# githubpradeep/llm_np_cp

Hardware: AMD Instinct MI355X
Metric: decode tokens/sec (higher is better)
Workload: dtype bf16; 1 GPU; model=llama-3.2-1b, kv_dtype=bf16, global_batch=1, seq_len=867, parallelism=tp1

## Files before the change

### csrc/llm_ops.hip

```cpp

#include <hip/hip_runtime.h>
#include <cstdint>
#include <cstdio>
#include <cstdlib>
#include <type_traits>

#include "common.h"


#define GEMV_ROWS_PER_BLOCK 4
#define STAGE_RAW 0
#define STAGE_NORM 1
#define STAGE_GLU 2
#define STAGE_NORM2 3
#define STAGE_NORM_EMBED 4

DEVINL u16 glu_act(float xx, float u, int act) {
  float a;
  if (act == 0) {
    a = xx / (1.f + __expf(-xx));
  } else {
    float c = 0.7978845608028654f * (xx + 0.044715f * xx * xx * xx);
    a = 0.5f * xx * (1.f + tanhf(c));
  }
// ... 1643 lines not shown
      sc[w] = (mls[w * 2] == -INFINITY) ? 0.f : __expf(mls[w * 2] - mt);
      lt += mls[w * 2 + 1] * sc[w];
    }
    float inv = 1.f / lt;
    for (int d = lane; d < hd; d += 64) {
      float v = 0.f;
#pragma unroll
      for (int w = 0; w < 4; w++) v += accs[w * hd + d] * sc[w];
      out[((size_t)m * nh + h) * hd + d] = f2b(v * inv);
    }
  }
}


template <bool KV8>
DEVINL void attn_dec_body(char* smem, const int chunk, const int SPLIT,
                          const u16* __restrict__ qkv, void* __restrict__ kc,
                          void* __restrict__ vc, u16* __restrict__ out,
                          const int* __restrict__ len_ptr,
                          const float* __restrict__ cost,
                          const float* __restrict__ sint,
                          float* __restrict__ kS, float* __restrict__ vS,
                          float* __restrict__ scratch, int* __restrict__ cnt,
                          int nh, int kvh, int hd, int S, float scale,
                          float softcap, int window) {
  float* red = (float*)smem;
  int* lastflag = (int*)(red + 4 * hd + 8);

  const int h = blockIdx.x;
  const int b = blockIdx.z;
  qkv += (size_t)b * (nh + 2 * kvh) * hd;
  out += (size_t)b * nh * hd;
  kc = (char*)kc + (size_t)b * kvh * S * hd * (KV8 ? 1 : 2);
  vc = (char*)vc + (size_t)b * kvh * S * hd * (KV8 ? 1 : 2);
  if (KV8) { kS += (size_t)b * kvh * S; vS += (size_t)b * kvh * S; }
  scratch += (size_t)b * nh * SPLIT * (hd + 2);
  cnt += b * nh;
  const int grp = nh / kvh;
  const int kvhead = h / grp;
  const int pos = len_ptr[b];
  int start = 0;
  if (window > 0 && pos + 1 - window > 0) start = pos + 1 - window;
  const int hist = pos - start;
  const int clen = (hist + SPLIT - 1) / SPLIT;
  const int c0 = start + chunk * clen;
  const int c1 = min(c0 + clen, pos);
  const bool last_chunk = (chunk == SPLIT - 1);

  const int LP = hd / 8;
  const int PP = 64 / LP;
  const int wave = threadIdx.x >> 6, lane = threadIdx.x & 63;
  const int p = lane / LP, d0 = (lane % LP) * 8;
  const int hd2 = hd / 2;
  const float* cp = cost + (size_t)pos * hd2;
  const float* sp = sint + (size_t)pos * hd2;

  const u16* qh = qkv + (size_t)h * hd;
  const u16* kh = qkv + (size_t)(nh + kvhead) * hd;
  const u16* vh = qkv + (size_t)(nh + kvh + kvhead) * hd;
  const u16* K0 = (const u16*)kc + (size_t)kvhead * S * hd;
  const u16* V0 = (const u16*)vc + (size_t)kvhead * S * hd;
  const uint8_t* K08 = (const uint8_t*)kc + (size_t)kvhead * S * hd;
  const uint8_t* V08 = (const uint8_t*)vc + (size_t)kvhead * S * hd;
  const float* kS0 = KV8 ? kS + (size_t)kvhead * S : nullptr;
  const float* vS0 = KV8 ? vS + (size_t)kvhead * S : nullptr;

// ... 174 lines not shown
    mrun = mn;
  }

  float* accs = red;
  float* mls = red + 4 * hd;
  if (lane < LP) {
#pragma unroll
    for (int j = 0; j < 8; j++) accs[wave * hd + d0 + j] = acc[j];
  }
  if (lane == 0) {
    mls[wave * 2] = mrun;
    mls[wave * 2 + 1] = lrun;
  }
  __syncthreads();

  float* part = scratch + ((size_t)h * SPLIT + chunk) * (hd + 2);
  if (wave == 0) {
    float mt = fmaxf(fmaxf(mls[0], mls[2]), fmaxf(mls[4], mls[6]));
    float lt = 0.f, sc[4];
#pragma unroll
    for (int w = 0; w < 4; w++) {
      sc[w] = (mls[w * 2] == -INFINITY) ? 0.f : __expf(mls[w * 2] - mt);
      lt += mls[w * 2 + 1] * sc[w];
    }
    if (SPLIT == 1) {
      float inv = 1.f / lt;
      for (int d = lane; d < hd; d += 64) {
        float v = 0.f;
#pragma unroll
        for (int w = 0; w < 4; w++) v += accs[w * hd + d] * sc[w];
        out[(size_t)h * hd + d] = f2b(v * inv);
      }
    } else {
      for (int d = lane; d < hd; d += 64) {
        float v = 0.f;
#pragma unroll
        for (int w = 0; w < 4; w++) v += accs[w * hd + d] * sc[w];
        part[2 + d] = v;
      }
      if (lane == 0) { part[0] = mt; part[1] = lt; }
    }
  }
  if (SPLIT == 1) return;

  asm volatile("s_waitcnt vmcnt(0)" ::: "memory");
  __syncthreads();
  if (threadIdx.x == 0) {
    __builtin_amdgcn_fence(__ATOMIC_RELEASE, "agent");
    asm volatile("s_waitcnt vmcnt(0)" ::: "memory");
    int t = __hip_atomic_fetch_add(&cnt[h], 1, __ATOMIC_RELAXED,
                                   __HIP_MEMORY_SCOPE_AGENT);
    *lastflag = (t == SPLIT - 1);
  }
  __syncthreads();
  if (!*lastflag) return;

  if (threadIdx.x == 0)
    __builtin_amdgcn_fence(__ATOMIC_ACQUIRE, "agent");
  __syncthreads();
  if (wave == 0) {
    const float* base = scratch + (size_t)h * SPLIT * (hd + 2);
    float mt = -INFINITY;
    for (int c = 0; c < SPLIT; c++)
      mt = fmaxf(mt, base[(size_t)c * (hd + 2)]);
    float lt = 0.f;
    for (int c = 0; c < SPLIT; c++) {
      float mc = base[(size_t)c * (hd + 2)];
      if (mc != -INFINITY)
        lt += base[(size_t)c * (hd + 2) + 1] * __expf(mc - mt);
    }
    float inv = 1.f / lt;
    for (int d = lane; d < hd; d += 64) {
      float v = 0.f;
      for (int c = 0; c < SPLIT; c++) {
        float mc = base[(size_t)c * (hd + 2)];
        if (mc != -INFINITY)
          v += base[(size_t)c * (hd + 2) + 2 + d] * __expf(mc - mt);
      }
      out[(size_t)h * hd + d] = f2b(v * inv);
    }
  }
  __syncthreads();
  if (threadIdx.x == 0) cnt[h] = 0;
}


struct AttnPf {
  const void* ptr[4];
  long bytes[4];
  long stride0;
  float* sink;
  int never;
};

constexpr int PF_LD = 8;
constexpr int PF_TRIP = 256 * PF_LD;

template <typename F>
// ... 2 lines not shown
#pragma unroll
  for (int j = 0; j < PF_LD; j++) {
    long s = seg(j * 256 + (int)threadIdx.x);
    s = s < nseg ? s : nseg - 1;
    v[j] = base[s];
  }
  uint32_t a = 0;
#pragma unroll
  for (int j = 0; j < PF_LD; j++) {
    asm volatile("" ::"v"(v[j]));
    a ^= v[j][0];
  }
  return a;
}

DEVINL void attn_dec_prefetch(const AttnPf& pf, const int split) {
  const uint32_t nx = gridDim.x;
  const uint32_t pfy = gridDim.y - split;
  const uint32_t npb = nx * pfy * gridDim.z;
  const uint32_t pb =
      (blockIdx.z * pfy + (blockIdx.y - split)) * nx + blockIdx.x;
  uint32_t acc = 0;
  uint32_t g0 = 0;
#pragma unroll
  for (int r = 0; r < 4; r++) {
    const u4v* base = (const u4v*)pf.ptr[r];
    const long nseg = pf.bytes[r] >> 4;
    if (base == nullptr || nseg <= 0) continue;
    const long spu = pf.stride0 >> 4;
    if (r == 0 && spu > 0 && (nx & 7) == 0 && nseg < (1l << 31)) {
      const uint32_t c = blockIdx.x & 7;
      const uint32_t nunit = (uint32_t)((nseg + spu - 1) / spu);
      if (nunit <= c) continue;
      const uint32_t uspu = (uint32_t)spu;
      const long vseg = (long)((nunit - c + 7) / 8) * spu;
      const uint32_t rc = (pb / nx) * (nx / 8) + blockIdx.x / 8;
// ... 36 lines not shown
  extern __shared__ __attribute__((aligned(16))) char smem[];
  int SPLIT = gridDim.y;
  if constexpr (PF) {
    const AttnPfLaunch& a = (pfa, ...);
    if ((int)blockIdx.y >= a.split) {
      attn_dec_prefetch(a.pf, a.split);
      return;
    }
    SPLIT = a.split;
  }
  attn_dec_body<KV8>(smem, blockIdx.y, SPLIT, qkv, kc, vc, out, len_ptr, cost,
                     sint, kS, vS, scratch, cnt, nh, kvh, hd, S, scale,
                     softcap, window);
}

static hipError_t attn_dec_launch(const void* qkv, void* kc, void* vc,
                                  void* out, const void* len_ptr,
                                  const void* cost, const void* sint,
                                  void* kS, void* vS, int kv8, void* scratch,
                                  void* cnt, int split, int batch, int nh,
                                  int kvh, int hd, int S, float scale,
                                  float softcap, int window, int pf_blocks,
                                  const AttnPf& pf, hipStream_t stream) {
  size_t lds = (4 * hd + 8) * sizeof(float) + 16;
  const int pfy = pf_blocks > 0 ? (pf_blocks + nh - 1) / nh : 0;
#define ATTN_DEC_ARGS                                                        \
  (const u16*)qkv, kc, vc, (u16*)out, (const int*)len_ptr,                   \
      (const float*)cost, (const float*)sint, (float*)kS, (float*)vS,        \
      (float*)scratch, (int*)cnt, nh, kvh, hd, S, scale, softcap, window
#define ATTN_DEC_CASE(KV8V)                                                  \
  hipLaunchKernelGGL((k_attn_dec_t<KV8V, false>), dim3(nh, split, batch),    \
                     dim3(256), lds, stream, ATTN_DEC_ARGS)
#define ATTN_DEC_PF_CASE(KV8V)                                               \
  hipLaunchKernelGGL((k_attn_dec_t<KV8V, true, AttnPfLaunch>),               \
                     dim3(nh, split + pfy, batch), dim3(256), lds, stream,   \
                     ATTN_DEC_ARGS, AttnPfLaunch{split, pf})
  if (pfy > 0) {
    if (kv8) ATTN_DEC_PF_CASE(true);
    else ATTN_DEC_PF_CASE(false);
  } else {
    if (kv8) ATTN_DEC_CASE(true);
    else ATTN_DEC_CASE(false);
  }
#undef ATTN_DEC_PF_CASE
#undef ATTN_DEC_ARGS
#undef ATTN_DEC_CASE
  return hipGetLastError();
}

extern "C" hipError_t launch_attn_dec_pf(
    const void* qkv, void* kc, void* vc, void* out, const void* len_ptr,
    const void* cost, const void* sint, void* kS, void* vS, int kv8,
    void* scratch, void* cnt, int split, int batch, int nh, int kvh, int hd,
    int S, float scale, float softcap, int window, int pf_blocks,
    const void* p0, long n0, const void* p1, long n1, const void* p2,
    long n2, const void* p3, long n3, long stride0, void* sink,
    hipStream_t stream) {
  AttnPf pf{{p0, p1, p2, p3}, {n0, n1, n2, n3}, stride0, (float*)sink, -1};
  if (pf_blocks > 0 && sink == nullptr) return hipErrorInvalidValue;
  return attn_dec_launch(qkv, kc, vc, out, len_ptr, cost, sint, kS, vS, kv8,
                         scratch, cnt, split, batch, nh, kvh, hd, S, scale,
                         softcap, window, pf_blocks, pf, stream);
}

extern "C" hipError_t launch_attn_dec(const void* qkv, void* kc, void* vc,
                                      void* out, const void* len_ptr,
                                      const void* cost, const void* sint,
                                      void* kS, void* vS, int kv8,
                                      void* scratch, void* cnt, int split,
                                      int batch,
                                      int nh, int kvh, int hd, int S,
                                      float scale, float softcap, int window,
                                      hipStream_t stream) {
  return attn_dec_launch(qkv, kc, vc, out, len_ptr, cost, sint, kS, vS, kv8,
                         scratch, cnt, split, batch, nh, kvh, hd, S, scale,
                         softcap, window, 0, AttnPf{}, stream);
}


typedef short b4v __attribute__((ext_vector_type(4)));

template <int HD, bool KV8>
__global__ void __launch_bounds__(64)
k_attn_prefill_mfma(const u16* __restrict__ q, const void* __restrict__ kc,
                    const void* __restrict__ vc, u16* __restrict__ out,
                    const int* __restrict__ len_ptr,
                    const float* __restrict__ kS,
                    const float* __restrict__ vS, int M, int nh, int kvh,
                    int S, float scale, float softcap, int window) {
  constexpr int HD32 = HD / 32;
  constexpr int HD16 = HD / 16;
// ... 240 lines not shown
DEVINL uint32_t fkey(float f) {
  union { float f; uint32_t u; } c; c.f = f;
  return (c.u & 0x80000000u) ? ~c.u : (c.u ^ 0x80000000u);
}
DEVINL float fkey_inv(uint32_t k) {
  union { float f; uint32_t u; } c;
  c.u = (k & 0x80000000u) ? (k ^ 0x80000000u) : ~k;
  return c.f;
}

DEVINL uint64_t pack_ki(uint32_t key, int idx) {
  return ((uint64_t)key << 32) | (uint32_t)(0x7fffffff - idx);
}
DEVINL int unpack_idx(uint64_t p) { return 0x7fffffff - (int)(uint32_t)p; }

DEVINL void logit_max_body(const void* __restrict__ logits, int V, int lbf16,
                           unsigned long long* __restrict__ gmax) {
  const int b = blockIdx.y;
  gmax += b;
  const float* lf = (const float*)logits + (size_t)b * V;
  const u16* lh = (const u16*)logits + (size_t)b * V;
  float mv = -INFINITY;
  int mi = 0;
  for (int i = blockIdx.x * 256 + threadIdx.x; i < V; i += gridDim.x * 256) {
    float v = lbf16 ? b2f(lh[i]) : lf[i];
    if (v > mv || (v == mv && i < mi)) { mv = v; mi = i; }
  }
  uint64_t pk = pack_ki(fkey(mv), mi);
#pragma unroll
  for (int w = 1; w < 64; w <<= 1) {
    uint64_t o = __shfl_xor((unsigned long long)pk, w);
    if (o > pk) pk = o;
  }
  __shared__ unsigned long long ws[4];
  if ((threadIdx.x & 63) == 0) ws[threadIdx.x >> 6] = pk;
  __syncthreads();
  if (threadIdx.x == 0) {
    uint64_t b = ws[0];
    for (int w = 1; w < 4; w++) if (ws[w] > b) b = ws[w];
    atomicMax(gmax, (unsigned long long)b);
  }
}
// ... 94 lines not shown
  gmax += b; pick += b; cnt += b; nout += b;
  out_ring += (size_t)b * ring_stride;
  const float* lf = (const float*)logits + (size_t)b * V;
  const u16* lh = (const u16*)logits + (size_t)b * V;
  float thresh = -INFINITY;
  uint32_t tau = 0;
  if (SEL) {
    sel += (size_t)b * SEL_WORDS;
    tau = (uint32_t)sel[SEL_TAU];
  } else if (!greedy) {
    thresh = fkey_inv((uint32_t)(*gmax >> 32)) + __logf(min_p) / inv_temp;
  }
  const uint32_t c = (uint32_t)(*ctr) ^ ((uint32_t)b * 0x85ebca6bu);
  float bv = -INFINITY;
  int bi = 0x7fffffff;
  for (int i = blockIdx.x * 256 + threadIdx.x; i < V; i += gridDim.x * 256) {
    float v = lbf16 ? b2f(lh[i]) : lf[i];
    if (SEL ? (fkey(v) < tau) : (v < thresh)) continue;
    float sc = v;
    if (!greedy) {
      uint32_t r = hash32(hash32((uint32_t)i ^ (c * 0x9e3779b9u)) ^
                          (uint32_t)seed);
      float u = (r + 1.0f) * 2.3283064e-10f;
      sc = v * inv_temp - __logf(-__logf(u));
    }
    if (sc > bv || (sc == bv && i < bi)) { bv = sc; bi = i; }
  }
  sample_pick_commit(bv, bi, V, gmax, pick, cnt, next_token, out_ring, nout,
                     len_ptr, bump_len, SEL ? sel : nullptr);
}

extern "C" __global__ void __launch_bounds__(256)
k_sample_pick(const void* __restrict__ logits, int V, int lbf16,
              long ring_stride, float min_p,
              int greedy, uint64_t seed, float inv_temp,
              unsigned long long* __restrict__ gmax,
              uint64_t* __restrict__ ctr,
              unsigned long long* __restrict__ pick,
              int* __restrict__ cnt, int* __restrict__ next_token,
              int* __restrict__ out_ring, int* __restrict__ nout,
              int* __restrict__ len_ptr, int bump_len) {
  sample_pick_body<false>(logits, V, lbf16, ring_stride, min_p, greedy, seed,
// ... 46 lines not shown
             __logf(__uint_as_float(samp[SAMP_MINP])) / inv_temp;
  if (MINP && selected) {
    const float min_p = __uint_as_float(samp[SAMP_MINP]);
    if (min_p > 0.0f) {
      float cut = fkey_inv((uint32_t)(*gmax >> 32)) + __logf(min_p) / inv_temp;
      if (cut == 0.0f) cut = -0.0f;
      const uint32_t kc = fkey(cut);
      if (kc > tau) tau = kc;
    }
  }
  const uint32_t k0 =
      hash32(hash32(samp[SAMP_CTR] ^ 0x9e3779b9u) ^ samp[SAMP_SEED]);
  const uint32_t k1 = hash32(k0 ^ samp[SAMP_SEED + 1] ^ 0x85ebca6bu);
  float bv = -INFINITY;
  int bi = 0x7fffffff;
  for (int i = blockIdx.x * 256 + threadIdx.x; i < V; i += gridDim.x * 256) {
    float v = lbf16 ? b2f(lh[i]) : lf[i];
    if (selected ? (fkey(v) < tau) : (v < thresh)) continue;
    float sc = v;
    if (!greedy) {
      uint32_t r = hash32(hash32((uint32_t)i ^ k0) ^ k1);
      float u = (r + 1.0f) * 2.3283064e-10f;
      sc = v * inv_temp - __logf(-__logf(u));
    }
    if (sc > bv || (sc == bv && i < bi)) { bv = sc; bi = i; }
  }
  sample_pick_commit(bv, bi, V, gmax, pick, cnt, next_token, out_ring, nout,
                     len_ptr, bump_len, selected ? sel : nullptr);
}

template <bool PHASE2>
DEVINL void sample_select_body(
    const void* __restrict__ logits, int V, int lbf16,
    int top_k, float top_p, float inv_temp, int shift,
    int last, const unsigned long long* __restrict__ gmax,
    unsigned long long* __restrict__ sel) {
  const int b = blockIdx.y;
  const int t = threadIdx.x;
  sel += (size_t)b * SEL_WORDS;
  unsigned long long* hist = sel + SEL_HIST;
  const float* lf = (const float*)logits + (size_t)b * V;
// ... 108 lines not shown
}

extern "C" __global__ void __launch_bounds__(256)
k_sample_select_rows2(const void* __restrict__ logits, int V, int lbf16,
                      const uint32_t* __restrict__ samp, int shift, int last,
                      const unsigned long long* __restrict__ gmax,
                      unsigned long long* __restrict__ sel) {
  samp += (size_t)blockIdx.y * SAMP_WORDS;
  const float top_p = __uint_as_float(samp[SAMP_TOPP]);
  if (samp[SAMP_MODE] != 2u || !(top_p < 1.0f)) return;
  sample_select_body<true>(logits, V, lbf16, 0, top_p,
                           __uint_as_float(samp[SAMP_INVT]), shift, last,
                           gmax, sel);
}

extern "C" hipError_t launch_sample(const void* logits, int V, int lbf16,
                                    int batch, long ring_stride, float min_p,
                                    int greedy, uint64_t seed, float inv_temp,
                                    void* ctr, void* gmax, void* pick,
                                    void* cnt, void* next_token,
                                    void* out_ring, void* nout,
                                    void* len_ptr, int bump_len,
                                    hipStream_t stream) {
  int blocks = (V + 255) / 256;
  if (blocks > 512) blocks = 512;
  if (batch > 1) {
    blocks = blocks / batch + 1;
    if (blocks < 16) blocks = 16;
  }
  if (!greedy)
    hipLaunchKernelGGL(k_logit_max, dim3(blocks, batch), dim3(256), 0,
                       stream, logits, V, lbf16, (unsigned long long*)gmax,
                       (uint64_t*)ctr);
  hipLaunchKernelGGL(k_sample_pick, dim3(blocks, batch), dim3(256), 0,
                     stream, logits, V, lbf16, ring_stride, min_p, greedy,
                     seed, inv_temp,
                     (unsigned long long*)gmax, (uint64_t*)ctr,
                     (unsigned long long*)pick, (int*)cnt, (int*)next_token,
                     (int*)out_ring, (int*)nout, (int*)len_ptr, bump_len);
  return hipGetLastError();
}

extern "C" hipError_t launch_sample_sel(
    const void* logits, int V, int lbf16, int batch, long ring_stride,
    float min_p, int greedy, uint64_t seed, float inv_temp, void* ctr,
    void* gmax, void* pick, void* cnt, void* next_token, void* out_ring,
    void* nout, void* len_ptr, int bump_len, int top_k, float top_p,
    void* sel, hipStream_t stream) {
  if (greedy || (top_k <= 0 && !(top_p < 1.0f)))
    return launch_sample(logits, V, lbf16, batch, ring_stride, min_p, greedy,
                         seed, inv_temp, ctr, gmax, pick, cnt, next_token,
                         out_ring, nout, len_ptr, bump_len, stream);
  if (top_k > V) top_k = V;
  int blocks = (V + 255) / 256;
  if (blocks > 512) blocks = 512;
  if (batch > 1) {
    blocks = blocks / batch + 1;
    if (blocks < 16) blocks = 16;
  }
  int sblocks = (V + 2047) / 2048;
  if (sblocks > 64) sblocks = 64;
  hipLaunchKernelGGL(k_logit_max, dim3(blocks, batch), dim3(256), 0, stream,
                     logits, V, lbf16, (unsigned long long*)gmax,
                     (uint64_t*)ctr);
  const int last_shift = lbf16 ? 16 : 0;
  for (int shift = 24; shift >= last_shift; shift -= 8)
    hipLaunchKernelGGL(k_sample_select, dim3(sblocks, batch), dim3(256), 0,
                       stream, logits, V, lbf16, top_k, top_p, inv_temp,
                       shift, shift == last_shift ? 1 : 0,
                       (const unsigned long long*)gmax,
                       (unsigned long long*)sel);
  hipLaunchKernelGGL(k_sample_pick_sel, dim3(blocks, batch), dim3(256), 0,
                     stream, logits, V, lbf16, ring_stride, seed, inv_temp,
                     (unsigned long long*)gmax, (uint64_t*)ctr,
                     (unsigned long long*)pick, (int*)cnt, (int*)next_token,
                     (int*)out_ring, (int*)nout, (int*)len_ptr, bump_len,
                     (unsigned long long*)sel);
  return hipGetLastError();
}

extern "C" hipError_t launch_sample_rows(
    const void* logits, int V, int lbf16, int batch, long ring_stride,
    void* samp, int any_sampled, int any_select, int chain, void* gmax,
    void* pick, void* cnt, void* next_token, void* out_ring, void* nout,
    void* len_ptr, int bump_len, void* sel, hipStream_t stream) {
  int blocks = (V + 255) / 256;
  if (blocks > 512) blocks = 512;
  if (batch > 1) {
    blocks = blocks / batch + 1;
    if (blocks < 16) blocks = 16;
  }
  if (!any_sampled && !any_select) {
    hipLaunchKernelGGL(k_sample_pick, dim3(blocks, batch), dim3(256), 0,
                       stream, logits, V, lbf16, ring_stride, 0.0f, 1,
                       (uint64_t)0, 1.0f, (unsigned long long*)gmax,
                       (uint64_t*)samp, (unsigned long long*)pick, (int*)cnt,
                       (int*)next_token, (int*)out_ring, (int*)nout,
                       (int*)len_ptr, bump_len);
    return hipGetLastError();
  }
  hipLaunchKernelGGL(k_logit_max_rows, dim3(blocks, batch), dim3(256), 0,
                     stream, logits, V, lbf16, (unsigned long long*)gmax,
                     (uint32_t*)samp);
  if (any_select) {
    int sblocks = (V + 2047) / 2048;
    if (sblocks > 64) sblocks = 64;
// ... 1524 lines not shown
```

### llm_np_cp_amd/models/engine.py

```python

from __future__ import annotations

import gc
from functools import partial
from typing import Dict, Optional

import numpy as np
import torch

from ..core.config import ModelConfig
from ..ops import hip_ops as ho
from ..parallel import tp as tpu
from ..utils.tracing import trace_range
from .decode_spec import RowState, SampleSpec


class DeviceCacheHandle:

    def __init__(self, engine):
        self.engine = engine
        self.seq_len = 0


class GPUModel:
# ... 364 lines not shown
        if self.moe:
            E = cfg.num_local_experts
            self.moe_idx = torch.zeros(PC * self.topk, dtype=torch.int32,
                                       device=dev)
            self.moe_w = torch.zeros(PC * self.topk, dtype=torch.float32,
                                     device=dev)
            self.moe_dense = torch.zeros(PC * E, dtype=torch.float32,
                                         device=dev)
        self.b_hb = torch.zeros(H, **bf)
        self.b_t2 = torch.zeros(H, **bf)
        self.b_gu = torch.zeros(2 * I, **bf)
        import os as _os
        _sp = _os.environ.get("LLM_ATTN_SPLIT")
        self.attn_split = (int(_sp) if _sp else
                           min(16, max(2, self.max_seq // 512)))
        self.attn_scratch = torch.zeros(
            self.nh_l * self.attn_split * (hd + 2), dtype=torch.float32,
            device=dev)
        self.attn_cnt = torch.zeros(self.nh_l, dtype=torch.int32, device=dev)
        self.s_gmax = torch.zeros(1, dtype=torch.int64, device=dev)
        self.s_pick = torch.zeros(1, dtype=torch.int64, device=dev)
        self.s_cnt = torch.zeros(1, dtype=torch.int32, device=dev)
        self.s_sel = torch.zeros(1, ho.SAMPLE_SEL_WORDS, dtype=torch.int64,
                                 device=dev)
        i32 = dict(dtype=torch.int32, device=dev)
        self.ids_buf = torch.zeros(PC, **i32)
        self.next_token = torch.zeros(1, **i32)
        self.out_ring = torch.zeros(max(65536, S + 16), **i32)
        self.nout = torch.zeros(1, **i32)
        self.len_buf = torch.zeros(1, **i32)
# ... 129 lines not shown
        if layer_hook is not None:
            layer_hook(-1, h[:M])
        for i, lw in enumerate(self.layers):
            window = cfg.sliding_window if cfg.is_sliding(i) else 0
            ho.rmsnorm(h[:M], lw["g_in"], xn[:M], eps=eps)
            if batch_attn:
                self._linear(lw, "wqkv", xn, self.bt_qkv, M=M)
                if "bqkv" in lw:
                    ho.bias_add(self.bt_qkv, lw["bqkv"], M)
                ho.attn_dec(self.bt_qkv, self.k_cache[i], self.v_cache[i],
                            self.b_att[0], self.bt_lens, self.cos_t,
                            self.sin_t, self.bt_scratch, self.bt_attn_cnt,
                            self.nh_l, self.kvh_l, self.hd, self.scale,
                            softcap=self.attn_softcap, window=window or 0,
                            split=self.attn_split, kS=self.k_scale[i],
                            vS=self.v_scale[i], batch=M)
            else:
                self._linear(lw, "wq", xn, self.b_q, M=M)
                self._linear(lw, "wk", xn, self.b_k, M=M)
                self._linear(lw, "wv", xn, self.b_v, M=M)
                if "bqkv" in lw:
                    ho.bias_add(self.b_q, lw["bias_q"], M)
                    ho.bias_add(self.b_k, lw["bias_k"], M)
                    ho.bias_add(self.b_v, lw["bias_v"], M)
                ho.rope_cache(self.b_q, self.b_k, self.b_v, self._kc(i),
                              self._vc(i), self.cos_t, self.sin_t,
                              self.len_buf, M, self.nh_l, self.kvh_l,
                              self.hd, kS=self._ks(i), vS=self._vs(i))
                if self.hd in (64, 128, 256):
                    ho.attn_prefill_mfma(
                        self.b_q, self._kc(i), self._vc(i), self.b_att,
# ... 776 lines not shown
                            g=lw["g_in"], res=lw.get("bqkv"), eps=eps)
            prev = lw
            pfkw = {}
            attn_dec = ho.attn_dec
            if self._attn_pf is not None and self._attn_pf[i]:
                attn_dec = ho.attn_dec_pf
                pfkw = dict(regions=self._attn_pf[i],
                            pf_blocks=self.attn_pf_blocks,
                            stride0=self.attn_pf_stride,
                            sink=self._pf_sink)
            attn_dec(self.b_qkv, self.k_cache[i], self.v_cache[i],
                     self.b_att[0], self.len_buf, self.cos_t, self.sin_t,
                     self.attn_scratch, self.attn_cnt,
                     self.nh_l, self.kvh_l, self.hd, self.scale,
                     softcap=self.attn_softcap, window=window or 0,
                     split=self.attn_split,
                     kS=self.k_scale[i], vS=self.v_scale[i], **pfkw)
            if self.gemma:
                self._dgemv(lw, "wo", self.b_att[0], t1)
                tpu.all_reduce(t1)
                self._dgemv(lw, "wgu", t1, self.b_gu, stage=ho.STAGE_NORM2,
                            x2=h, g=lw["g_post"], g2=lw["g_preffn"],
                            res=hnext, eps=eps, **gukw)
                h, hnext = hnext, h
                self._dgemv(lw, "wdown", self.b_gu[:self.inter_l], t2,
                            **downkw)
                tpu.all_reduce(t2)
            else:
                if self.tp_branch:
                    self._dgemv(lw, "wo", self.b_att[0], t1)
                    tpu.all_reduce(t1)
# ... 123 lines not shown
                x, xstride = self.embed, 0
                st = dict(stage=ho.STAGE_NORM_EMBED, x2=self.bt_next,
                          g=lw["g_in"], hout=h, hstride=H, eps=eps,
                          escale=cfg.embed_scale)
            else:
                st = dict(stage=ho.STAGE_NORM, g=lw["g_in"], eps=eps)
            proj(lw["wqkv_q"], lw["wqkv_s"], x, xstride, self.bt_qkv, H,
                 qkvw, bias=lw.get("bqkv"), **st)
            prev = lw
            ho.attn_dec(self.bt_qkv, self.k_cache[i], self.v_cache[i],
                        self.b_att[0], self.bt_lens, self.cos_t, self.sin_t,
                        self.bt_scratch, self.bt_attn_cnt,
                        self.nh_l, self.kvh_l, self.hd, self.scale,
                        softcap=self.attn_softcap, window=window or 0,
                        split=self.attn_split, kS=self.k_scale[i],
                        vS=self.v_scale[i], batch=B)
            if self.gemma:
                proj(lw["wo_q"], lw["wo_s"], self.b_att, nhh, t1, nhh, H)
                proj(lw["wgu_q"], lw["wgu_s"], t1, H, gu, H, 2 * I,
                     **norm2(lw["g_post"], lw["g_preffn"]))
                h, hb = hb, h
                proj(lw["wdown_q"], lw["wdown_s"], gu, 2 * I, t2, I, H,
                     **glu)
            else:
                proj(lw["wo_q"], lw["wo_s"], self.b_att, nhh, h, nhh, H,
                     res=h)
                proj(lw["wgu_q"], lw["wgu_s"], h, H, gu, H, 2 * I,
                     stage=ho.STAGE_NORM, g=lw["g_post"], eps=eps)
                proj(lw["wdown_q"], lw["wdown_s"], gu, 2 * I, h, I, H,
                     res=h, **glu)
        if self.gemma:
# ... 312 lines not shown
```

### llm_np_cp_amd/ops/hip_ops.py

```python

from __future__ import annotations

import ctypes
import os

import numpy as np
import torch

_LIB = None
_LIB_PATH = os.path.join(os.path.dirname(os.path.dirname(
    os.path.abspath(__file__))), "_libllmops.so")

_SIGS = {
    "launch_gemv_bf16": [ctypes.c_void_p] * 7 + [ctypes.c_int] * 4 +
                        [ctypes.c_float, ctypes.c_int, ctypes.c_float,
                         ctypes.c_int, ctypes.c_int, ctypes.c_int,
                         ctypes.c_float, ctypes.c_void_p, ctypes.c_long,
                         ctypes.c_void_p, ctypes.c_void_p, ctypes.c_int],
    "launch_gemv_fp8": [ctypes.c_void_p] * 8 + [ctypes.c_int] * 4 +
                       [ctypes.c_float, ctypes.c_int, ctypes.c_float,
                        ctypes.c_int, ctypes.c_int, ctypes.c_int,
                        ctypes.c_float, ctypes.c_void_p, ctypes.c_long,
                        ctypes.c_long, ctypes.c_void_p, ctypes.c_void_p],
    "launch_rmsnorm": [ctypes.c_void_p] * 4 + [ctypes.c_int] * 2 +
                      [ctypes.c_float, ctypes.c_int, ctypes.c_void_p],
    "launch_rope_cache": [ctypes.c_void_p] * 7 + [ctypes.c_int] +
                         [ctypes.c_void_p] * 3 + [ctypes.c_int] * 5 +
                         [ctypes.c_void_p],
    "launch_attn": [ctypes.c_void_p] * 7 + [ctypes.c_int] * 6 +
                   [ctypes.c_float, ctypes.c_float, ctypes.c_int,
                    ctypes.c_void_p],
    "launch_attn_prefill_mfma": [ctypes.c_void_p] * 7 + [ctypes.c_int] * 6 +
                                [ctypes.c_float, ctypes.c_float,
                                 ctypes.c_int, ctypes.c_void_p],
    "launch_attn_dec": [ctypes.c_void_p] * 9 + [ctypes.c_int] +
                       [ctypes.c_void_p] * 2 + [ctypes.c_int] * 6 +
                       [ctypes.c_float, ctypes.c_float, ctypes.c_int,
                        ctypes.c_void_p],
    "launch_attn_dec_pf": [ctypes.c_void_p] * 9 + [ctypes.c_int] +
                          [ctypes.c_void_p] * 2 + [ctypes.c_int] * 6 +
                          [ctypes.c_float, ctypes.c_float, ctypes.c_int,
                           ctypes.c_int] +
                          [ctypes.c_void_p, ctypes.c_long] * 4 +
                          [ctypes.c_long, ctypes.c_void_p, ctypes.c_void_p],
    "launch_glu": [ctypes.c_void_p] * 3 + [ctypes.c_long, ctypes.c_int,
                                           ctypes.c_void_p],
    "launch_embed": [ctypes.c_void_p] * 3 + [ctypes.c_int] * 2 +
                    [ctypes.c_float, ctypes.c_void_p],
    "launch_sample": [ctypes.c_void_p, ctypes.c_int, ctypes.c_int,
                      ctypes.c_int, ctypes.c_long, ctypes.c_float,
                      ctypes.c_int, ctypes.c_uint64, ctypes.c_float] +
                     [ctypes.c_void_p] * 8 +
                     [ctypes.c_int, ctypes.c_void_p],
    "launch_sample_sel": [ctypes.c_void_p, ctypes.c_int, ctypes.c_int,
                          ctypes.c_int, ctypes.c_long, ctypes.c_float,
                          ctypes.c_int, ctypes.c_uint64, ctypes.c_float] +
                         [ctypes.c_void_p] * 8 +
                         [ctypes.c_int, ctypes.c_int, ctypes.c_float,
                          ctypes.c_void_p, ctypes.c_void_p],
    "launch_sample_rows": [ctypes.c_void_p, ctypes.c_int, ctypes.c_int,
                           ctypes.c_int, ctypes.c_long, ctypes.c_void_p,
                           ctypes.c_int, ctypes.c_int, ctypes.c_int] +
                          [ctypes.c_void_p] * 7 +
                          [ctypes.c_int, ctypes.c_void_p, ctypes.c_void_p],
    "launch_logit_adjust": [ctypes.c_void_p, ctypes.c_int, ctypes.c_int,
                            ctypes.c_int] + [ctypes.c_void_p] * 4 +
                           [ctypes.c_int, ctypes.c_void_p],
    "launch_tokstat_mark": [ctypes.c_void_p, ctypes.c_void_p, ctypes.c_int,
# ... 197 lines not shown

def attn_prefill_mfma(q: torch.Tensor, k_cache: torch.Tensor,
                      v_cache: torch.Tensor, out: torch.Tensor,
                      len_ptr: torch.Tensor, M: int, nh: int, kvh: int,
                      hd: int, scale: float, softcap: float = 0.0,
                      window: int = 0, kS: torch.Tensor | None = None,
                      vS: torch.Tensor | None = None):
    S = k_cache.shape[1]
    _check(lib().launch_attn_prefill_mfma(
        _ptr(q), _ptr(k_cache), _ptr(v_cache), _ptr(out), _ptr(len_ptr),
        _ptr(kS), _ptr(vS), 1 if kS is not None else 0,
        M, nh, kvh, hd, S, ctypes.c_float(scale), ctypes.c_float(softcap),
        window, _stream()), "attn_prefill_mfma")


def attn_dec(qkv: torch.Tensor, k_cache: torch.Tensor,
             v_cache: torch.Tensor, out: torch.Tensor,
             len_ptr: torch.Tensor, cos_t: torch.Tensor,
             sin_t: torch.Tensor, scratch: torch.Tensor,
             cnt: torch.Tensor, nh: int, kvh: int, hd: int,
             scale: float, softcap: float = 0.0, window: int = 0,
             split: int = 1, kS: torch.Tensor | None = None,
             vS: torch.Tensor | None = None, batch: int = 1):
    S = k_cache.shape[-2]
    _check(lib().launch_attn_dec(
        _ptr(qkv), _ptr(k_cache), _ptr(v_cache), _ptr(out), _ptr(len_ptr),
        _ptr(cos_t), _ptr(sin_t), _ptr(kS), _ptr(vS),
        1 if kS is not None else 0,
        _ptr(scratch), _ptr(cnt), split, batch,
        nh, kvh, hd, S, ctypes.c_float(scale),
        ctypes.c_float(softcap), window, _stream()), "attn_dec")


def attn_dec_pf(qkv: torch.Tensor, k_cache: torch.Tensor,
                v_cache: torch.Tensor, out: torch.Tensor,
                len_ptr: torch.Tensor, cos_t: torch.Tensor,
                sin_t: torch.Tensor, scratch: torch.Tensor,
                cnt: torch.Tensor, nh: int, kvh: int, hd: int,
                scale: float, softcap: float = 0.0, window: int = 0,
                split: int = 1, kS: torch.Tensor | None = None,
                vS: torch.Tensor | None = None, batch: int = 1, *,
                regions=(), pf_blocks: int = 0, stride0: int = 0,
                sink: torch.Tensor | None = None):
    S = k_cache.shape[-2]
    regions = list(regions)
    assert len(regions) <= 4
    if pf_blocks > 0:
        assert sink is not None and sink.numel() >= 256
    flat = []
    for addr, nbytes in regions + [(0, 0)] * (4 - len(regions)):
        assert addr % 16 == 0 and nbytes >= 0
        flat += [addr, nbytes]
    _check(lib().launch_attn_dec_pf(
        _ptr(qkv), _ptr(k_cache), _ptr(v_cache), _ptr(out), _ptr(len_ptr),
        _ptr(cos_t), _ptr(sin_t), _ptr(kS), _ptr(vS),
        1 if kS is not None else 0,
        _ptr(scratch), _ptr(cnt), split, batch,
        nh, kvh, hd, S, ctypes.c_float(scale),
        ctypes.c_float(softcap), window, pf_blocks, *flat, stride0,
        _ptr(sink), _stream()), "attn_dec_pf")


def glu(gate: torch.Tensor, up: torch.Tensor, out: torch.Tensor, act: int):
    total = gate.numel()
    assert total % 8 == 0
    _check(lib().launch_glu(_ptr(gate), _ptr(up), _ptr(out), total, act,
                            _stream()), "glu")


def embed(table: torch.Tensor, ids: torch.Tensor, out: torch.Tensor,
          M: int, scale: float = 1.0):
    H = table.shape[1]
    _check(lib().launch_embed(_ptr(table), _ptr(ids), _ptr(out), M, H,
                              ctypes.c_float(scale), _stream()), "embed")


SAMPLE_SEL_WORDS = 260


def sample(logits: torch.Tensor, min_p: float, greedy: bool, seed: int,
           ctr: torch.Tensor, gmax: torch.Tensor, pick: torch.Tensor,
           next_token: torch.Tensor, out_ring: torch.Tensor,
           nout: torch.Tensor, len_ptr: torch.Tensor,
           bump_len: bool = True, temperature: float = 1.0,
           cnt: torch.Tensor | None = None, batch: int = 1, *,
           top_k: int = 0, top_p: float = 1.0,
           sel: torch.Tensor | None = None):
    if top_k < 0:
        raise ValueError(f"top_k must be >= 0, got {top_k}")
    if not 0.0 < top_p <= 1.0:
        raise ValueError(f"top_p must be in (0, 1], got {top_p}")
    filtered = top_k > 0 or top_p < 1.0
    if filtered and greedy:
        raise ValueError("top_k / top_p do not combine with greedy")
    if top_k > 0 and top_p < 1.0:
        raise ValueError("top_k and top_p are separate strategies; "
                         "pass one of them")
    if filtered and (sel is None or sel.dtype != torch.int64
                     or sel.numel() < batch * SAMPLE_SEL_WORDS):
        raise ValueError(f"top_k / top_p need an int64 `sel` scratch of "
                         f"{SAMPLE_SEL_WORDS} words per row")
    V = logits.shape[-1]
# ... 19 lines not shown
        _check(lib().launch_sample_sel(
            _ptr(logits), V, lbf16, batch, ctypes.c_long(ring_stride),
            ctypes.c_float(min_p), 0,
            ctypes.c_uint64(seed), ctypes.c_float(inv_temp),
            _ptr(ctr), _ptr(gmax), _ptr(pick), _ptr(cnt),
            _ptr(next_token), _ptr(out_ring), _ptr(nout), _ptr(len_ptr),
            1 if bump_len else 0, int(top_k), ctypes.c_float(top_p),
            _ptr(sel), _stream()), "sample_sel")
        return
    _check(lib().launch_sample(
        _ptr(logits), V, lbf16, batch, ctypes.c_long(ring_stride),
        ctypes.c_float(min_p), 1 if greedy else 0,
        ctypes.c_uint64(seed), ctypes.c_float(inv_temp),
        _ptr(ctr), _ptr(gmax), _ptr(pick), _ptr(cnt),
        _ptr(next_token), _ptr(out_ring), _ptr(nout), _ptr(len_ptr),
        1 if bump_len else 0, _stream()), "sample")


SAMP_WORDS = 8
SAMP_GREEDY, SAMP_MIN_P, SAMP_TOP_K, SAMP_TOP_P = 0, 1, 2, 3
SAMP_CTR = 7


def samp_row(params, seed: int, V: int) -> np.ndarray:
    V = int(V)
    if V <= 0:
        raise ValueError(f"V must be positive, got {V}")
    strategy = params.get("strategy", "min_p")
    temperature = float(params.get("temperature", 1.0))
    if not temperature == temperature:
        raise ValueError("temperature must not be NaN")
# ... 596 lines not shown
```

Before: 1380 tokens/s.

## Merge split-K decode attention chunks inside one block instead of atomic ticket

Adds a block-merge decode attention path. All split chunks of a head run as wave groups inside one larger workgroup (256*SPLIT threads), write their partials to LDS, and are merged after a __syncthreads. This replaces the global scratch, release/acquire fences and atomic ticket counter. It is the default ('auto') when split is 2-4, at the cost of fewer, larger blocks and therefore less grid parallelism. Separately, the logits scans in sampling now use vectorized 16-byte loads, and the sample pick launches fewer blocks (one per 1024 vocab entries, capped at 64 instead of up to 512).

```diff
diff --git a/csrc/llm_ops.hip b/csrc/llm_ops.hip
--- a/csrc/llm_ops.hip
+++ b/csrc/llm_ops.hip
@@ -1681,19 +1681,17 @@
 
 
 template <bool KV8>
-DEVINL void attn_dec_body(char* smem, const int chunk, const int SPLIT,
-                          const u16* __restrict__ qkv, void* __restrict__ kc,
-                          void* __restrict__ vc, u16* __restrict__ out,
-                          const int* __restrict__ len_ptr,
-                          const float* __restrict__ cost,
-                          const float* __restrict__ sint,
-                          float* __restrict__ kS, float* __restrict__ vS,
-                          float* __restrict__ scratch, int* __restrict__ cnt,
-                          int nh, int kvh, int hd, int S, float scale,
-                          float softcap, int window) {
-  float* red = (float*)smem;
-  int* lastflag = (int*)(red + 4 * hd + 8);
-
+DEVINL void attn_dec_chunk(float* red, const int chunk, const int SPLIT,
+                           const int wave, const int lane,
+                           float* __restrict__ parts, const int pidx,
+                           const u16* __restrict__ qkv, void* __restrict__ kc,
+                           void* __restrict__ vc, u16* __restrict__ out,
+                           const int* __restrict__ len_ptr,
+                           const float* __restrict__ cost,
+                           const float* __restrict__ sint,
+                           float* __restrict__ kS, float* __restrict__ vS,
+                           int nh, int kvh, int hd, int S, float scale,
+                           float softcap, int window) {
   const int h = blockIdx.x;
   const int b = blockIdx.z;
   qkv += (size_t)b * (nh + 2 * kvh) * hd;
@@ -1701,8 +1699,6 @@
   kc = (char*)kc + (size_t)b * kvh * S * hd * (KV8 ? 1 : 2);
   vc = (char*)vc + (size_t)b * kvh * S * hd * (KV8 ? 1 : 2);
   if (KV8) { kS += (size_t)b * kvh * S; vS += (size_t)b * kvh * S; }
-  scratch += (size_t)b * nh * SPLIT * (hd + 2);
-  cnt += b * nh;
   const int grp = nh / kvh;
   const int kvhead = h / grp;
   const int pos = len_ptr[b];
@@ -1716,7 +1712,6 @@
 
   const int LP = hd / 8;
   const int PP = 64 / LP;
-  const int wave = threadIdx.x >> 6, lane = threadIdx.x & 63;
   const int p = lane / LP, d0 = (lane % LP) * 8;
   const int hd2 = hd / 2;
   const float* cp = cost + (size_t)pos * hd2;
@@ -1921,7 +1916,7 @@
   }
   __syncthreads();
 
-  float* part = scratch + ((size_t)h * SPLIT + chunk) * (hd + 2);
+  float* part = parts + (size_t)pidx * (hd + 2);
   if (wave == 0) {
     float mt = fmaxf(fmaxf(mls[0], mls[2]), fmaxf(mls[4], mls[6]));
     float lt = 0.f, sc[4];
@@ -1948,6 +1943,52 @@
       if (lane == 0) { part[0] = mt; part[1] = lt; }
     }
   }
+}
+
+DEVINL void attn_dec_merge(const float* base, const int SPLIT, const int lane,
+                           const int hd, u16* out_h) {
+  float mt = -INFINITY;
+  for (int c = 0; c < SPLIT; c++)
+    mt = fmaxf(mt, base[(size_t)c * (hd + 2)]);
+  float lt = 0.f;
+  for (int c = 0; c < SPLIT; c++) {
+    float mc = base[(size_t)c * (hd + 2)];
+    if (mc != -INFINITY)
+      lt += base[(size_t)c * (hd + 2) + 1] * __expf(mc - mt);
+  }
+  float inv = 1.f / lt;
+  for (int d = lane; d < hd; d += 64) {
+    float v = 0.f;
+    for (int c = 0; c < SPLIT; c++) {
+      float mc = base[(size_t)c * (hd + 2)];
+      if (mc != -INFINITY)
+        v += base[(size_t)c * (hd + 2) + 2 + d] * __expf(mc - mt);
+    }
+    out_h[d] = f2b(v * inv);
+  }
+}
+
+template <bool KV8>
+DEVINL void attn_dec_body(char* smem, const int chunk, const int SPLIT,
+                          const u16* __restrict__ qkv, void* __restrict__ kc,
+                          void* __restrict__ vc, u16* __restrict__ out,
+                          const int* __restrict__ len_ptr,
+                          const float* __restrict__ cost,
+                          const float* __restrict__ sint,
+                          float* __restrict__ kS, float* __restrict__ vS,
+                          float* __restrict__ scratch, int* __restrict__ cnt,
+                          int nh, int kvh, int hd, int S, float scale,
+                          float softcap, int window) {
+  float* red = (float*)smem;
+  int* lastflag = (int*)(red + 4 * hd + 8);
+  const int h = blockIdx.x;
+  const int b = blockIdx.z;
+  scratch += (size_t)b * nh * SPLIT * (hd + 2);
+  cnt += b * nh;
+  const int wave = threadIdx.x >> 6, lane = threadIdx.x & 63;
+  attn_dec_chunk<KV8>(red, chunk, SPLIT, wave, lane, scratch,
+                      h * SPLIT + chunk, qkv, kc, vc, out, len_ptr, cost,
+                      sint, kS, vS, nh, kvh, hd, S, scale, softcap, window);
   if (SPLIT == 1) return;
 
   asm volatile("s_waitcnt vmcnt(0)" ::: "memory");
@@ -1965,30 +2006,34 @@
   if (threadIdx.x == 0)
     __builtin_amdgcn_fence(__ATOMIC_ACQUIRE, "agent");
   __syncthreads();
-  if (wave == 0) {
-    const float* base = scratch + (size_t)h * SPLIT * (hd + 2);
-    float mt = -INFINITY;
-    for (int c = 0; c < SPLIT; c++)
-      mt = fmaxf(mt, base[(size_t)c * (hd + 2)]);
-    float lt = 0.f;
-    for (int c = 0; c < SPLIT; c++) {
-      float mc = base[(size_t)c * (hd + 2)];
-      if (mc != -INFINITY)
-        lt += base[(size_t)c * (hd + 2) + 1] * __expf(mc - mt);
-    }
-    float inv = 1.f / lt;
-    for (int d = lane; d < hd; d += 64) {
-      float v = 0.f;
-      for (int c = 0; c < SPLIT; c++) {
-        float mc = base[(size_t)c * (hd + 2)];
-        if (mc != -INFINITY)
-          v += base[(size_t)c * (hd + 2) + 2 + d] * __expf(mc - mt);
-      }
-      out[(size_t)h * hd + d] = f2b(v * inv);
-    }
-  }
+  if (wave == 0)
+    attn_dec_merge(scratch + (size_t)h * SPLIT * (hd + 2), SPLIT, lane, hd,
+                   out + ((size_t)b * nh + h) * hd);
   __syncthreads();
   if (threadIdx.x == 0) cnt[h] = 0;
+}
+
+template <bool KV8, int SPLIT>
+DEVINL void attn_dec_body_blk(char* smem, const u16* __restrict__ qkv,
+                              void* __restrict__ kc, void* __restrict__ vc,
+                              u16* __restrict__ out,
+                              const int* __restrict__ len_ptr,
+                              const float* __restrict__ cost,
+                              const float* __restrict__ sint,
+                              float* __restrict__ kS, float* __restrict__ vS,
+                              int nh, int kvh, int hd, int S, float scale,
+                              float softcap, int window) {
+  const int wg = threadIdx.x >> 6, lane = threadIdx.x & 63;
+  const int chunk = wg >> 2;
+  float* red = (float*)smem + chunk * (4 * hd + 8);
+  float* parts = (float*)smem + SPLIT * (4 * hd + 8);
+  attn_dec_chunk<KV8>(red, chunk, SPLIT, wg & 3, lane, parts, chunk,
+                      qkv, kc, vc, out, len_ptr, cost, sint, kS, vS, nh, kvh,
+                      hd, S, scale, softcap, window);
+  __syncthreads();
+  if (wg == 0)
+    attn_dec_merge(parts, SPLIT, lane, hd,
+                   out + ((size_t)blockIdx.z * nh + blockIdx.x) * hd);
 }
 
 
@@ -2021,12 +2066,12 @@
   return a;
 }
 
-DEVINL void attn_dec_prefetch(const AttnPf& pf, const int split) {
+DEVINL void attn_dec_prefetch(const AttnPf& pf, const int arows) {
   const uint32_t nx = gridDim.x;
-  const uint32_t pfy = gridDim.y - split;
+  const uint32_t pfy = gridDim.y - arows;
   const uint32_t npb = nx * pfy * gridDim.z;
   const uint32_t pb =
-      (blockIdx.z * pfy + (blockIdx.y - split)) * nx + blockIdx.x;
+      (blockIdx.z * pfy + (blockIdx.y - arows)) * nx + blockIdx.x;
   uint32_t acc = 0;
   uint32_t g0 = 0;
 #pragma unroll
@@ -2093,6 +2138,31 @@
                      softcap, window);
 }
 
+template <bool KV8, int SPLIT, bool PF, typename... PFA>
+__global__ void __launch_bounds__(256 * SPLIT)
+k_attn_dec_blk_t(const u16* __restrict__ qkv, void* __restrict__ kc,
+                 void* __restrict__ vc, u16* __restrict__ out,
+                 const int* __restrict__ len_ptr,
+                 const float* __restrict__ cost,
+                 const float* __restrict__ sint, float* __restrict__ kS,
+                 float* __restrict__ vS, int nh, int kvh, int hd, int S,
+                 float scale, float softcap, int window, PFA... pfa) {
+  static_assert(sizeof...(PFA) == (PF ? 1 : 0), "PF takes one AttnPf");
+  static_assert(SPLIT >= 2 && SPLIT <= 4, "256 * SPLIT threads, one block");
+  extern __shared__ __attribute__((aligned(16))) char smem[];
+  if constexpr (PF) {
+    if (blockIdx.y >= 1) {
+      if (threadIdx.x >= 256) return;
+      const AttnPf& pf = (pfa, ...);
+      attn_dec_prefetch(pf, 1);
+      return;
+    }
+  }
+  attn_dec_body_blk<KV8, SPLIT>(smem, qkv, kc, vc, out, len_ptr, cost, sint,
+                                kS, vS, nh, kvh, hd, S, scale, softcap,
+                                window);
+}
+
 static hipError_t attn_dec_launch(const void* qkv, void* kc, void* vc,
                                   void* out, const void* len_ptr,
                                   const void* cost, const void* sint,
@@ -2100,9 +2170,43 @@
                                   void* cnt, int split, int batch, int nh,
                                   int kvh, int hd, int S, float scale,
                                   float softcap, int window, int pf_blocks,
-                                  const AttnPf& pf, hipStream_t stream) {
+                                  const AttnPf& pf, int merge,
+                                  hipStream_t stream) {
+  if (merge < 0 || merge > 2 || split < 1) return hipErrorInvalidValue;
+  if (merge == 2 && 256 * split > 1024) return hipErrorInvalidValue;
   size_t lds = (4 * hd + 8) * sizeof(float) + 16;
   const int pfy = pf_blocks > 0 ? (pf_blocks + nh - 1) / nh : 0;
+  if (merge != 1 && split >= 2 && split <= 4) {
+    const size_t blds =
+        (size_t)split * ((4 * hd + 8) + (hd + 2)) * sizeof(float);
+#define ATTN_BLK_ARGS                                                        \
+  (const u16*)qkv, kc, vc, (u16*)out, (const int*)len_ptr,                   \
+      (const float*)cost, (const float*)sint, (float*)kS, (float*)vS, nh,    \
+      kvh, hd, S, scale, softcap, window
+#define ATTN_BLK_CASE(KV8V, SP)                                              \
+  do {                                                                       \
+    if (pfy > 0)                                                             \
+      hipLaunchKernelGGL((k_attn_dec_blk_t<KV8V, SP, true, AttnPf>),         \
+                         dim3(nh, 1 + pfy, batch), dim3(256 * SP), blds,     \
+                         stream, ATTN_BLK_ARGS, pf);                         \
+    else                                                                     \
+      hipLaunchKernelGGL((k_attn_dec_blk_t<KV8V, SP, false>),                \
+                         dim3(nh, 1, batch), dim3(256 * SP), blds, stream,   \
+                         ATTN_BLK_ARGS);                                     \
+  } while (0)
+#define ATTN_BLK_SPLIT(KV8V)                                                 \
+  do {                                                                       \
+    if (split == 2) ATTN_BLK_CASE(KV8V, 2);                                  \
+    else if (split == 3) ATTN_BLK_CASE(KV8V, 3);                             \
+    else ATTN_BLK_CASE(KV8V, 4);                                             \
+  } while (0)
+    if (kv8) ATTN_BLK_SPLIT(true);
+    else ATTN_BLK_SPLIT(false);
+#undef ATTN_BLK_SPLIT
+#undef ATTN_BLK_CASE
+#undef ATTN_BLK_ARGS
+    return hipGetLastError();
+  }
 #define ATTN_DEC_ARGS                                                        \
   (const u16*)qkv, kc, vc, (u16*)out, (const int*)len_ptr,                   \
       (const float*)cost, (const float*)sint, (float*)kS, (float*)vS,        \
@@ -2133,13 +2237,13 @@
     void* scratch, void* cnt, int split, int batch, int nh, int kvh, int hd,
     int S, float scale, float softcap, int window, int pf_blocks,
     const void* p0, long n0, const void* p1, long n1, const void* p2,
-    long n2, const void* p3, long n3, long stride0, void* sink,
+    long n2, const void* p3, long n3, long stride0, void* sink, int merge,
     hipStream_t stream) {
   AttnPf pf{{p0, p1, p2, p3}, {n0, n1, n2, n3}, stride0, (float*)sink, -1};
   if (pf_blocks > 0 && sink == nullptr) return hipErrorInvalidValue;
   return attn_dec_launch(qkv, kc, vc, out, len_ptr, cost, sint, kS, vS, kv8,
                          scratch, cnt, split, batch, nh, kvh, hd, S, scale,
-                         softcap, window, pf_blocks, pf, stream);
+                         softcap, window, pf_blocks, pf, merge, stream);
 }
 
 extern "C" hipError_t launch_attn_dec(const void* qkv, void* kc, void* vc,
@@ -2150,10 +2254,10 @@
                                       int batch,
                                       int nh, int kvh, int hd, int S,
                                       float scale, float softcap, int window,
-                                      hipStream_t stream) {
+                                      int merge, hipStream_t stream) {
   return attn_dec_launch(qkv, kc, vc, out, len_ptr, cost, sint, kS, vS, kv8,
                          scratch, cnt, split, batch, nh, kvh, hd, S, scale,
-                         softcap, window, 0, AttnPf{}, stream);
+                         softcap, window, 0, AttnPf{}, merge, stream);
 }
 
 
@@ -2424,6 +2528,37 @@
 }
 DEVINL int unpack_idx(uint64_t p) { return 0x7fffffff - (int)(uint32_t)p; }
 
+template <typename F>
+DEVINL void logits_scan(const float* __restrict__ lf,
+                        const u16* __restrict__ lh, int V, int lbf16, F f) {
+  const int t = blockIdx.x * 256 + threadIdx.x;
+  const int nt = gridDim.x * 256;
+  int done = 0;
+  if (lbf16) {
+    if (((uintptr_t)lh & 15) == 0) {
+      const int nv = V >> 3;
+      for (int k = t; k < nv; k += nt) {
+        s8v x = ((const s8v*)lh)[k];
+#pragma unroll
+        for (int j = 0; j < 8; j++) f(k * 8 + j, b2f(((u16*)&x)[j]));
+      }
+      done = nv << 3;
+    }
+    for (int i = done + t; i < V; i += nt) f(i, b2f(lh[i]));
+  } else {
+    if (((uintptr_t)lf & 15) == 0) {
+      const int nv = V >> 2;
+      for (int k = t; k < nv; k += nt) {
+        f4v x = ((const f4v*)lf)[k];
+#pragma unroll
+        for (int j = 0; j < 4; j++) f(k * 4 + j, x[j]);
+      }
+      done = nv << 2;
+    }
+    for (int i = done + t; i < V; i += nt) f(i, lf[i]);
+  }
+}
+
 DEVINL void logit_max_body(const void* __restrict__ logits, int V, int lbf16,
                            unsigned long long* __restrict__ gmax) {
   const int b = blockIdx.y;
@@ -2432,10 +2567,9 @@
   const u16* lh = (const u16*)logits + (size_t)b * V;
   float mv = -INFINITY;
   int mi = 0;
-  for (int i = blockIdx.x * 256 + threadIdx.x; i < V; i += gridDim.x * 256) {
-    float v = lbf16 ? b2f(lh[i]) : lf[i];
+  logits_scan(lf, lh, V, lbf16, [&](int i, float v) {
     if (v > mv || (v == mv && i < mi)) { mv = v; mi = i; }
-  }
+  });
   uint64_t pk = pack_ki(fkey(mv), mi);
 #pragma unroll
   for (int w = 1; w < 64; w <<= 1) {
@@ -2560,9 +2694,8 @@
   const uint32_t c = (uint32_t)(*ctr) ^ ((uint32_t)b * 0x85ebca6bu);
   float bv = -INFINITY;
   int bi = 0x7fffffff;
-  for (int i = blockIdx.x * 256 + threadIdx.x; i < V; i += gridDim.x * 256) {
-    float v = lbf16 ? b2f(lh[i]) : lf[i];
-    if (SEL ? (fkey(v) < tau) : (v < thresh)) continue;
+  logits_scan(lf, lh, V, lbf16, [&](int i, float v) {
+    if (SEL ? (fkey(v) < tau) : (v < thresh)) return;
     float sc = v;
     if (!greedy) {
       uint32_t r = hash32(hash32((uint32_t)i ^ (c * 0x9e3779b9u)) ^
@@ -2571,7 +2704,7 @@
       sc = v * inv_temp - __logf(-__logf(u));
     }
     if (sc > bv || (sc == bv && i < bi)) { bv = sc; bi = i; }
-  }
+  });
   sample_pick_commit(bv, bi, V, gmax, pick, cnt, next_token, out_ring, nout,
                      len_ptr, bump_len, SEL ? sel : nullptr);
 }
@@ -2648,9 +2781,8 @@
   const uint32_t k1 = hash32(k0 ^ samp[SAMP_SEED + 1] ^ 0x85ebca6bu);
   float bv = -INFINITY;
   int bi = 0x7fffffff;
-  for (int i = blockIdx.x * 256 + threadIdx.x; i < V; i += gridDim.x * 256) {
-    float v = lbf16 ? b2f(lh[i]) : lf[i];
-    if (selected ? (fkey(v) < tau) : (v < thresh)) continue;
+  logits_scan(lf, lh, V, lbf16, [&](int i, float v) {
+    if (selected ? (fkey(v) < tau) : (v < thresh)) return;
     float sc = v;
     if (!greedy) {
       uint32_t r = hash32(hash32((uint32_t)i ^ k0) ^ k1);
@@ -2658,7 +2790,7 @@
       sc = v * inv_temp - __logf(-__logf(u));
     }
     if (sc > bv || (sc == bv && i < bi)) { bv = sc; bi = i; }
-  }
+  });
   sample_pick_commit(bv, bi, V, gmax, pick, cnt, next_token, out_ring, nout,
                      len_ptr, bump_len, selected ? sel : nullptr);
 }
@@ -2797,20 +2929,30 @@
                            gmax, sel);
 }
 
+constexpr int SAMPLE_PICK_SPAN = 1024;
+constexpr int SAMPLE_PICK_CAP = 64;
+static int sample_pick_blocks(int V, int batch, int blocks) {
+  if (blocks > 0) return blocks;
+  blocks = (V + SAMPLE_PICK_SPAN - 1) / SAMPLE_PICK_SPAN;
+  if (blocks > SAMPLE_PICK_CAP) blocks = SAMPLE_PICK_CAP;
+  if (batch > 1) {
+    const int floor_ = blocks < 16 ? blocks : 16;
+    blocks = blocks / batch + 1;
+    if (blocks < floor_) blocks = floor_;
+  }
+  return blocks < 1 ? 1 : blocks;
+}
+
 extern "C" hipError_t launch_sample(const void* logits, int V, int lbf16,
                                     int batch, long ring_stride, float min_p,
                                     int greedy, uint64_t seed, float inv_temp,
                                     void* ctr, void* gmax, void* pick,
                                     void* cnt, void* next_token,
                                     void* out_ring, void* nout,
-                                    void* len_ptr, int bump_len,
+                                    void* len_ptr, int bump_len, int blocks,
                                     hipStream_t stream) {
-  int blocks = (V + 255) / 256;
-  if (blocks > 512) blocks = 512;
-  if (batch > 1) {
-    blocks = blocks / batch + 1;
-    if (blocks < 16) blocks = 16;
-  }
+  if (blocks < 0 || blocks > 65535) return hipErrorInvalidValue;
+  blocks = sample_pick_blocks(V, batch, blocks);
   if (!greedy)
     hipLaunchKernelGGL(k_logit_max, dim3(blocks, batch), dim3(256), 0,
                        stream, logits, V, lbf16, (unsigned long long*)gmax,
@@ -2833,14 +2975,9 @@
   if (greedy || (top_k <= 0 && !(top_p < 1.0f)))
     return launch_sample(logits, V, lbf16, batch, ring_stride, min_p, greedy,
                          seed, inv_temp, ctr, gmax, pick, cnt, next_token,
-                         out_ring, nout, len_ptr, bump_len, stream);
+                         out_ring, nout, len_ptr, bump_len, 0, stream);
   if (top_k > V) top_k = V;
-  int blocks = (V + 255) / 256;
-  if (blocks > 512) blocks = 512;
-  if (batch > 1) {
-    blocks = blocks / batch + 1;
-    if (blocks < 16) blocks = 16;
-  }
+  const int blocks = sample_pick_blocks(V, batch, 0);
   int sblocks = (V + 2047) / 2048;
   if (sblocks > 64) sblocks = 64;
   hipLaunchKernelGGL(k_logit_max, dim3(blocks, batch), dim3(256), 0, stream,
@@ -2867,12 +3004,7 @@
     void* samp, int any_sampled, int any_select, int chain, void* gmax,
     void* pick, void* cnt, void* next_token, void* out_ring, void* nout,
     void* len_ptr, int bump_len, void* sel, hipStream_t stream) {
-  int blocks = (V + 255) / 256;
-  if (blocks > 512) blocks = 512;
-  if (batch > 1) {
-    blocks = blocks / batch + 1;
-    if (blocks < 16) blocks = 16;
-  }
+  const int blocks = sample_pick_blocks(V, batch, 0);
   if (!any_sampled && !any_select) {
     hipLaunchKernelGGL(k_sample_pick, dim3(blocks, batch), dim3(256), 0,
                        stream, logits, V, lbf16, ring_stride, 0.0f, 1,
diff --git a/llm_np_cp_amd/models/engine.py b/llm_np_cp_amd/models/engine.py
--- a/llm_np_cp_amd/models/engine.py
+++ b/llm_np_cp_amd/models/engine.py
@@ -402,6 +402,11 @@
         _sp = _os.environ.get("LLM_ATTN_SPLIT")
         self.attn_split = (int(_sp) if _sp else
                            min(16, max(2, self.max_seq // 512)))
+        self.attn_merge = _os.environ.get("LLM_ATTN_MERGE") or "auto"
+        if self.attn_merge not in ho.ATTN_MERGE:
+            raise ValueError(f"LLM_ATTN_MERGE must be one of "
+                             f"{sorted(ho.ATTN_MERGE)}, got "
+                             f"{self.attn_merge!r}")
         self.attn_scratch = torch.zeros(
             self.nh_l * self.attn_split * (hd + 2), dtype=torch.float32,
             device=dev)
@@ -561,7 +566,8 @@
                             self.nh_l, self.kvh_l, self.hd, self.scale,
                             softcap=self.attn_softcap, window=window or 0,
                             split=self.attn_split, kS=self.k_scale[i],
-                            vS=self.v_scale[i], batch=M)
+                            vS=self.v_scale[i], batch=M,
+                            merge=self.attn_merge)
             else:
                 self._linear(lw, "wq", xn, self.b_q, M=M)
                 self._linear(lw, "wk", xn, self.b_k, M=M)
@@ -1368,7 +1374,7 @@
                      self.attn_scratch, self.attn_cnt,
                      self.nh_l, self.kvh_l, self.hd, self.scale,
                      softcap=self.attn_softcap, window=window or 0,
-                     split=self.attn_split,
+                     split=self.attn_split, merge=self.attn_merge,
                      kS=self.k_scale[i], vS=self.v_scale[i], **pfkw)
             if self.gemma:
                 self._dgemv(lw, "wo", self.b_att[0], t1)
@@ -1522,7 +1528,7 @@
                         self.nh_l, self.kvh_l, self.hd, self.scale,
                         softcap=self.attn_softcap, window=window or 0,
                         split=self.attn_split, kS=self.k_scale[i],
-                        vS=self.v_scale[i], batch=B)
+                        vS=self.v_scale[i], batch=B, merge=self.attn_merge)
             if self.gemma:
                 proj(lw["wo_q"], lw["wo_s"], self.b_att, nhh, t1, nhh, H)
                 proj(lw["wgu_q"], lw["wgu_s"], t1, H, gu, H, 2 * I,
diff --git a/llm_np_cp_amd/ops/hip_ops.py b/llm_np_cp_amd/ops/hip_ops.py
--- a/llm_np_cp_amd/ops/hip_ops.py
+++ b/llm_np_cp_amd/ops/hip_ops.py
@@ -36,13 +36,14 @@
     "launch_attn_dec": [ctypes.c_void_p] * 9 + [ctypes.c_int] +
                        [ctypes.c_void_p] * 2 + [ctypes.c_int] * 6 +
                        [ctypes.c_float, ctypes.c_float, ctypes.c_int,
-                        ctypes.c_void_p],
+                        ctypes.c_int, ctypes.c_void_p],
     "launch_attn_dec_pf": [ctypes.c_void_p] * 9 + [ctypes.c_int] +
                           [ctypes.c_void_p] * 2 + [ctypes.c_int] * 6 +
                           [ctypes.c_float, ctypes.c_float, ctypes.c_int,
                            ctypes.c_int] +
                           [ctypes.c_void_p, ctypes.c_long] * 4 +
-                          [ctypes.c_long, ctypes.c_void_p, ctypes.c_void_p],
+                          [ctypes.c_long, ctypes.c_void_p, ctypes.c_int,
+                           ctypes.c_void_p],
     "launch_glu": [ctypes.c_void_p] * 3 + [ctypes.c_long, ctypes.c_int,
                                            ctypes.c_void_p],
     "launch_embed": [ctypes.c_void_p] * 3 + [ctypes.c_int] * 2 +
@@ -51,7 +52,7 @@
                       ctypes.c_int, ctypes.c_long, ctypes.c_float,
                       ctypes.c_int, ctypes.c_uint64, ctypes.c_float] +
                      [ctypes.c_void_p] * 8 +
-                     [ctypes.c_int, ctypes.c_void_p],
+                     [ctypes.c_int, ctypes.c_int, ctypes.c_void_p],
     "launch_sample_sel": [ctypes.c_void_p, ctypes.c_int, ctypes.c_int,
                           ctypes.c_int, ctypes.c_long, ctypes.c_float,
                           ctypes.c_int, ctypes.c_uint64, ctypes.c_float] +
@@ -279,6 +280,16 @@
         window, _stream()), "attn_prefill_mfma")
 
 
+ATTN_MERGE = {"auto": 0, "ticket": 1, "block": 2}
+
+
+def _attn_merge(merge: str) -> int:
+    if merge not in ATTN_MERGE:
+        raise ValueError(f"merge must be one of {sorted(ATTN_MERGE)}, "
+                         f"got {merge!r}")
+    return ATTN_MERGE[merge]
+
+
 def attn_dec(qkv: torch.Tensor, k_cache: torch.Tensor,
              v_cache: torch.Tensor, out: torch.Tensor,
              len_ptr: torch.Tensor, cos_t: torch.Tensor,
@@ -286,7 +297,8 @@
              cnt: torch.Tensor, nh: int, kvh: int, hd: int,
              scale: float, softcap: float = 0.0, window: int = 0,
              split: int = 1, kS: torch.Tensor | None = None,
-             vS: torch.Tensor | None = None, batch: int = 1):
+             vS: torch.Tensor | None = None, batch: int = 1, *,
+             merge: str = "auto"):
     S = k_cache.shape[-2]
     _check(lib().launch_attn_dec(
         _ptr(qkv), _ptr(k_cache), _ptr(v_cache), _ptr(out), _ptr(len_ptr),
@@ -294,7 +306,8 @@
         1 if kS is not None else 0,
         _ptr(scratch), _ptr(cnt), split, batch,
         nh, kvh, hd, S, ctypes.c_float(scale),
-        ctypes.c_float(softcap), window, _stream()), "attn_dec")
+        ctypes.c_float(softcap), window, _attn_merge(merge), _stream()),
+        "attn_dec")
 
 
 def attn_dec_pf(qkv: torch.Tensor, k_cache: torch.Tensor,
@@ -306,7 +319,7 @@
                 split: int = 1, kS: torch.Tensor | None = None,
                 vS: torch.Tensor | None = None, batch: int = 1, *,
                 regions=(), pf_blocks: int = 0, stride0: int = 0,
-                sink: torch.Tensor | None = None):
+                sink: torch.Tensor | None = None, merge: str = "auto"):
     S = k_cache.shape[-2]
     regions = list(regions)
     assert len(regions) <= 4
@@ -323,7 +336,7 @@
         _ptr(scratch), _ptr(cnt), split, batch,
         nh, kvh, hd, S, ctypes.c_float(scale),
         ctypes.c_float(softcap), window, pf_blocks, *flat, stride0,
-        _ptr(sink), _stream()), "attn_dec_pf")
+        _ptr(sink), _attn_merge(merge), _stream()), "attn_dec_pf")
 
 
 def glu(gate: torch.Tensor, up: torch.Tensor, out: torch.Tensor, act: int):
@@ -350,7 +363,11 @@
            bump_len: bool = True, temperature: float = 1.0,
            cnt: torch.Tensor | None = None, batch: int = 1, *,
            top_k: int = 0, top_p: float = 1.0,
-           sel: torch.Tensor | None = None):
+           sel: torch.Tensor | None = None, blocks: int | None = None):
+    if blocks is not None and (top_k > 0 or top_p < 1.0):
+        raise ValueError("blocks applies to the min-p / greedy launch only")
+    if blocks is not None and blocks < 1:
+        raise ValueError(f"blocks must be >= 1, got {blocks}")
     if top_k < 0:
         raise ValueError(f"top_k must be >= 0, got {top_k}")
     if not 0.0 < top_p <= 1.0:
@@ -400,7 +417,7 @@
         ctypes.c_uint64(seed), ctypes.c_float(inv_temp),
         _ptr(ctr), _ptr(gmax), _ptr(pick), _ptr(cnt),
         _ptr(next_token), _ptr(out_ring), _ptr(nout), _ptr(len_ptr),
-        1 if bump_len else 0, _stream()), "sample")
+        1 if bump_len else 0, int(blocks or 0), _stream()), "sample")
 
 
 SAMP_WORDS = 8
```

Measured after the change: 1438 tokens/s, median of 6. +4.2%, better.
